# meilisearch/meilisearch

Measured on NVIDIA H100. Metric: queries/sec (batch=1024, typo-tolerant keyword + 768-d cosine hybrid search, semanticRatio 0.5, top-20), higher is better.
Workload: dtype u64+f16/f32

## Files before the change

include/b200milli.h:

```cpp
#ifndef B200MILLI_H
#define B200MILLI_H
#include <stdint.h>
#ifdef __cplusplus
extern "C" {
#endif

#define B200_OK 0
#define B200_ERR_NO_DEVICE (-1)
#define B200_ERR_CUDA (-2)
#define B200_ERR_INVALID (-3)
#define B200_ERR_UNSUPPORTED (-4)
#define B200_ERR_CAPACITY (-5)
#define B200_ERR_STATE (-6)

typedef struct b200_index b200_index;

int b200_open(int device_ordinal, b200_index **out);
void b200_close(b200_index *);
const char *b200_last_error(const b200_index *);
const char *b200_open_error(void);

enum b200_db {
    B200_DB_WORD_DOCIDS = 0,
    B200_DB_EXACT_WORD_DOCIDS = 1,
// ... 161 lines not shown
void b200_rule_end(b200_rule *);

enum b200_kernel { B200_K_LEV = 0, B200_K_COMPACT = 1, B200_K_PAIR_PROBE = 2, B200_K_SCATTER = 3, B200_K_EVAL_PATHS = 4, B200_K_EMIT = 5,
                   B200_K_VEC_DIST = 6, B200_K_TOPK = 7, B200_K_VEC_GEMM = 8, B200_K_VEC_MERGE = 9, B200_K_SORT = 10, B200_K_GEO = 11,
                   B200_K_GEO_FILTER = 12, B200_K_FACET = 13, B200_K_FACET_SEARCH = 14, B200_K_COUNT = 15 };
typedef struct {
    uint64_t kernel_launches;
    uint64_t device_steps;
    uint64_t posting_bytes;
    uint64_t matrix_bytes;
    uint64_t dictionary_bytes;
    uint64_t vector_bytes;
    double kernel_ms[B200_K_COUNT];
    uint64_t kernel_count[B200_K_COUNT];
    uint64_t kernel_bytes[B200_K_COUNT];
    double device_ms;
    uint64_t h2d_bytes, d2h_bytes;
    double host_ms[8];
    uint64_t hbm_bytes_staged;
    uint64_t deferred;
    uint64_t arena_peak_bytes;
    uint64_t eval_class_launches[9];
    uint64_t eval_class_tiles[9];
} b200_stats;
int b200_get_stats(b200_index *, b200_stats *out);
int b200_reset_stats(b200_index *);

#ifdef __cplusplus
}
#endif
#endif
```

meilisearch_b200/__init__.py:

```python
from __future__ import annotations

import ctypes as C
import os
import subprocess

import numpy as np

from .tokenizer import TokenBatch, tokenize

_HERE = os.path.dirname(os.path.abspath(__file__))
LIB_PATH = os.path.join(_HERE, "libb200milli.so")
MAX_SCORES = 12
CRITERIA = {"words": 0, "typo": 1, "proximity": 2, "attribute": 3, "attributeRank": 4, "wordPosition": 5, "sort": 6, "exactness": 7}
DEFAULT_CRITERIA = ["words", "typo", "proximity", "attributeRank", "sort", "wordPosition", "exactness"]
TMS = {"last": 0, "all": 1, "frequency": 2}
SCORE_KINDS = ["words", "typo", "proximity", "fid", "position", "exactAttribute", "exactWords", "vector", "skipped", "sort", "geo"]
GEO_STRATEGIES = {"dynamic": 0, "iterative": 1, "rtree": 2}
DB_FACET_F64, DB_FACET_STRING = 10, 11
DB_FACET_NORMALIZED, DB_FACET_ORIGINALS = 12, 13
NO_FIELD = 0xFFFF
ERRORS = {-1: "NO_DEVICE", -2: "CUDA", -3: "INVALID", -4: "UNSUPPORTED", -5: "CAPACITY", -6: "STATE"}


class B200Error(RuntimeError):
# ... 17 lines not shown
                ("ranking_score_threshold", C.c_double), ("sort_begin", C.c_void_p), ("sort_fid", C.c_void_p), ("sort_asc", C.c_void_p),
                ("sort_geo", C.c_void_p), ("sort_geo_point", C.c_void_p), ("geo_strategy", C.c_int32), ("geo_cache_size", C.c_uint32),
                ("geo_max_bucket_size", C.c_uint64), ("geo_filter_begin", C.c_void_p), ("geo_filter_kind", C.c_void_p),
                ("geo_filter_not", C.c_void_p), ("geo_filter_args", C.c_void_p), ("facet_begin", C.c_void_p), ("facet_fid", C.c_void_p),
                ("facet_order", C.c_void_p), ("facet_max_values", C.c_uint32), ("facet_cap", C.c_uint32), ("facet_search_fid", C.c_void_p),
                ("facet_query_kind", C.c_void_p), ("facet_query_off", C.c_void_p), ("facet_query_bytes", C.c_void_p),
                ("facet_search_flags", C.c_void_p), ("facet_search_max", C.c_uint32)]


class _Results(C.Structure):
    _fields_ = [(n, C.c_void_p) for n in ("docids", "n_hits", "n_scores", "score_kind", "score_rank", "score_max", "score_sim",
                                          "n_candidates", "semantic_hits", "status", "degraded", "used_negative_operator", "candidates")] + \
               [("candidates_words", C.c_uint64)] + \
               [(n, C.c_void_p) for n in ("facet_n_num", "facet_n_str", "facet_key", "facet_count", "facet_docid", "facet_has_stats", "facet_min",
                                          "facet_max")] + \
               [(n, C.c_void_p) for n in ("fs_n", "fs_key", "fs_count", "fs_docid", "fs_fallback")]


class _Stats(C.Structure):
    _fields_ = [("kernel_launches", C.c_uint64), ("device_steps", C.c_uint64), ("posting_bytes", C.c_uint64), ("matrix_bytes", C.c_uint64),
                ("dictionary_bytes", C.c_uint64), ("vector_bytes", C.c_uint64), ("kernel_ms", C.c_double * 15),
                ("kernel_count", C.c_uint64 * 15), ("kernel_bytes", C.c_uint64 * 15), ("device_ms", C.c_double), ("h2d_bytes", C.c_uint64), ("d2h_bytes", C.c_uint64), ("host_ms", C.c_double * 8),
                ("hbm_bytes_staged", C.c_uint64), ("deferred", C.c_uint64), ("arena_peak_bytes", C.c_uint64),
                ("eval_class_launches", C.c_uint64 * 9), ("eval_class_tiles", C.c_uint64 * 9)]


KERNELS = ["lev_match", "act_compact", "pair_probe", "scatter", "eval_paths", "emit", "vec_dist", "topk_select", "vec_gemm_topk", "vec_merge", "sort", "geo", "geo_filter", "facet", "facet_search"]


def build_library(force=False):
    csrc = os.path.join(_HERE, "csrc")
    srcs = [os.path.join(csrc, f) for f in os.listdir(csrc) if f.endswith((".cu", ".cpp", ".h"))] + [os.path.join(_HERE, "..", "include", "b200milli.h")]
    if force or not os.path.exists(LIB_PATH) or any(os.path.getmtime(s) > os.path.getmtime(LIB_PATH) for s in srcs):
        subprocess.check_call(["sh", os.path.join(csrc, "build.sh")])
    return LIB_PATH


_lib = None


def load_library():
    global _lib
    if _lib is None:
        if not os.path.exists(LIB_PATH):
            raise ImportError(f"{LIB_PATH} is missing: run `python -c 'import __graft_entry__ as g; g.build()'` (no CPU fallback exists)")
        l = C.CDLL(LIB_PATH)
        l.b200_open.argtypes = [C.c_int, C.POINTER(C.c_void_p)]
# ... 735 lines not shown
```

meilisearch_b200/csrc/device_types.h:

```cpp
#pragma once
#include <cstdint>

namespace b200 {

struct DListRef {
    unsigned long long off;
    uint32_t card;
    uint32_t dense;
};

constexpr int LEV_MAX_Q = 64;
constexpr int LEV_TERMS_PER_CTA = 32;
constexpr int LEV_REC_CAP = 2048;
struct LevTerm {
    uint8_t q[LEV_MAX_Q];
    uint8_t len;
    int8_t k_same;
    int8_t k_diff;
    uint8_t prefix;
};
struct LevRec {
    uint32_t base;
    uint32_t pad;
    unsigned long long codes;
};

constexpr uint32_t MAX_COSTS = 128;
constexpr uint32_t JOB_CHUNK = 2048;

struct DpState {
    uint32_t edge_begin;
    uint32_t pair_off;
    uint16_t n_edges;
    uint16_t rmin, rcount;
    uint16_t pad;
};
struct DpEdge {
    uint16_t dst;
    uint16_t cost;
    uint16_t col;
    uint16_t pad;
};
constexpr uint32_t MAX_WALK = 14;
struct PathOut {
    uint32_t act;
    uint16_t cost_idx;
    uint16_t len;
// ... 184 lines not shown
```

meilisearch_b200/csrc/engine.h:

```cpp
#pragma once
#include <cuda_runtime.h>

#include <chrono>
#include <condition_variable>
#include <functional>
#include <map>
#include <mutex>
#include <thread>
#include <atomic>
#include <memory>
#include <string>
#include <vector>

#include <sched.h>

#include "../../include/b200milli.h"
#include "device_types.h"
#include "host_index.h"
#include "query_model.h"

namespace b200 {

struct DeviceIndex {
    uint8_t *dict_bytes = nullptr;
// ... 375 lines not shown
    uint8_t *arena = nullptr;
    size_t arena_bytes = 0;
    uint8_t *scratch = nullptr;
    size_t scratch_bytes = 0;
    DevBuf<uint32_t> d_docids_out;
    DevBuf<SortDesc> d_sort_desc;
    DevBuf<uint32_t> d_sort_keys, d_sort_info;
    GeoPoint *d_geo_pts = nullptr;
    unsigned long long *d_geo_ub = nullptr;
    DevBuf<GeoCount> d_geo_count;
    DevBuf<GeoDesc> d_geo_desc;
    DevBuf<uint32_t> d_geo_u32;
    DevBuf<double> d_geo_dist;
    DevBuf<unsigned long long> d_geo_key;
    DevBuf<GeoClause> d_gf_clause;
    DevBuf<GeoFirst> d_gf_first;
    DevBuf<uint32_t> d_gf_u32;
    DevBuf<GeoSlot> d_gf_slot;
    DevBuf<unsigned long long> d_gf_count, d_gf_caller, d_gf_univ;
    DevBuf<unsigned long long> d_universes;
    DevBuf<uint32_t> d_rowtab;
    DevBuf<LevTerm> d_lev_terms;
    DevBuf<LevRec> d_lev_recs;
    DevBuf<uint32_t> d_lev_u32;
    DevBuf<float> d_vq, d_vdist, d_vsel_dist;
    DevBuf<uint32_t> d_vsel_ids, d_vsel_n;
    DevBuf<unsigned long long> d_cand, d_vruns, d_vpartial;
    DevBuf<uint16_t> d_vq16;
    std::vector<cudaEvent_t> ev_pool;
    struct Timed { int cls; size_t a, b; };
    std::vector<Timed> timed;
    size_t ev_used = 0;
    size_t mark();
    void time_kernel(int cls, size_t a, size_t b, uint64_t bytes) {
        timed.push_back(Timed{cls, a, b});
        stats.kernel_count[cls]++;
        stats.kernel_bytes[cls] += bytes;
        stats.kernel_launches++;
    }
    void resolve_timers();

    std::mutex err_mu;
    int fail(int code, const std::string &msg) {
        std::lock_guard<std::mutex> g(err_mu);
        last_error = msg;
        return code;
// ... 82 lines not shown
```

meilisearch_b200/csrc/engine_stage.cpp:

```cpp
#include <cuda_fp16.h>
#include <dlfcn.h>

#include <algorithm>
#include <cctype>
#include <cmath>
#include <cstdio>
#include <cstdlib>
#include <cstring>
#include <stdexcept>

#include "engine.h"
#include "kernels.h"

namespace b200 {

void HostAffinity::detect(int device) {
    valid = false;
    if (const char *env = getenv("B200_PIN"))
        if (atoi(env) == 0) return;
    char bus[32] = {};
    if (cudaDeviceGetPCIBusId(bus, sizeof bus, device) != cudaSuccess) return;
    for (char *c = bus; *c; c++) *c = (char)tolower((unsigned char)*c);
    int node = -1;
    {
// ... 75 lines not shown
    d_facet_out.release();
    d_facet_cand.release();
    if (d_geo_pts) cudaFree(d_geo_pts);
    if (d_geo_ub) cudaFree(d_geo_ub);
    d_geo_count.release();
    d_geo_desc.release();
    d_geo_u32.release();
    d_geo_dist.release();
    d_geo_key.release();
    d_gf_clause.release();
    d_gf_first.release();
    d_gf_u32.release();
    d_gf_slot.release();
    d_gf_count.release();
    d_gf_caller.release();
    d_gf_univ.release();
    for (auto &ln : lanes) ln.release();
    d_docids_out.release();
    d_sort_desc.release();
    d_sort_keys.release();
    d_sort_info.release();
    d_lev_terms.release();
    d_lev_recs.release();
    d_lev_u32.release();
    d_vq.release();
    d_vdist.release();
    d_vsel_dist.release();
    d_vsel_ids.release();
    d_vsel_n.release();
    d_cand.release();
    for (auto e : ev_pool) cudaEventDestroy(e);
    if (sc.comm && sc.comm_destroy) sc.comm_destroy(sc.comm);
    d_gather_ids.release();
    d_gather_dist.release();
    d_gather_n.release();
    for (auto e : vt.ev_pool) cudaEventDestroy(e);
    if (vt.stream) cudaStreamDestroy(vt.stream);
    if (stream) cudaStreamDestroy(stream);
}

size_t Engine::mark() {
    if (ev_used == ev_pool.size()) {
        cudaEvent_t e;
        cudaEventCreate(&e);
        ev_pool.push_back(e);
    }
    cudaEventRecord(ev_pool[ev_used], stream);
    return ev_used++;
}
void Engine::resolve_timers() {
    for (auto &t : timed) {
        float ms = 0;
        if (cudaEventElapsedTime(&ms, ev_pool[t.a], ev_pool[t.b]) == cudaSuccess) stats.kernel_ms[t.cls] += ms;
    }
    timed.clear();
    ev_used = 0;
}

int Engine::stage_finish() {
    CU(cudaSetDevice(device), "cudaSetDevice");
    try {
        build_host_index(raw_dict_bytes, raw_dict_off, raw_dbs, raw_docids, hix);
        build_sort_fields(raw_dbs[B200_DB_FACET_ID_F64_DOCIDS], raw_dbs[B200_DB_FACET_ID_STRING_DOCIDS], hix);
        build_geo_field(raw_dbs[B200_DB_FACET_ID_F64_DOCIDS], raw_dbs[B200_DB_FACET_ID_STRING_DOCIDS], hix);
        build_facet_search(raw_dbs[B200_DB_FACET_ID_STRING_DOCIDS], raw_dbs[B200_DB_FACET_ID_NORMALIZED_STRING_STRINGS],
                           raw_dbs[B200_DB_FIELD_ID_DOCID_FACET_STRINGS], hix);
    } catch (const std::exception &e) {
        return fail(B200_ERR_INVALID, e.what());
    }
    Settings keep = hix.settings;
    (void)keep;
    std::vector<uint32_t> off32(hix.dict_off.size());
    for (size_t i = 0; i < off32.size(); i++) off32[i] = (uint32_t)hix.dict_off[i];
    if (off32.empty()) off32.push_back(0);
    CU(upload(&dix.dict_bytes, hix.dict_bytes.data(), hix.dict_bytes.size()), "upload dictionary");
    CU(upload(&dix.dict_off, off32.data(), off32.size()), "upload dictionary offsets");
    CU(upload(&dix.pool, hix.pool.data(), hix.pool.size()), "upload posting pool");
    static_assert(sizeof(ListRef) == sizeof(DListRef), "ListRef layout");
    CU(upload(&dix.lists, reinterpret_cast<const DListRef *>(hix.lists.data()), hix.lists.size()), "upload list table");
    CU(upload(&dix.pair_keys, reinterpret_cast<const unsigned long long *>(hix.pair_keys.data()), hix.pair_keys.size()), "upload pair keys");
    CU(upload(&dix.base_ub, reinterpret_cast<const unsigned long long *>(hix.base_ub.data()), hix.base_ub.size()), "upload universe");
    stats.hbm_bytes_staged = hix.dict_bytes.size() + off32.size() * 4 + hix.pool.size() * 4 + hix.lists.size() * sizeof(ListRef) +
                             hix.pair_keys.size() * 8 + hix.base_ub.size() * 8;
    std::vector<uint32_t>().swap(hix.pool);
    for (auto &kv : hix.sort_fields)
// ... 114 lines not shown
        CU(cudaMemcpyAsync(dix.emb_docids, docids, n * 4, cudaMemcpyHostToDevice, stream), "H2D embedding docids");
    else {
        std::vector<uint32_t> ids(n);
        for (uint64_t r = 0; r < n; r++) ids[r] = (uint32_t)r;
        CU(cudaMemcpy(dix.emb_docids, ids.data(), n * 4, cudaMemcpyHostToDevice), "H2D embedding docids");
    }
    CU(cudaStreamSynchronize(stream), "sync");
    emb_bitmap.assign(hix.n_words64, 0);
    for (uint64_t r = 0; r < n; r++) {
        const uint32_t doc = docids ? docids[r] : (uint32_t)r;
        if ((doc >> 6) < emb_bitmap.size()) emb_bitmap[doc >> 6] |= 1ull << (doc & 63);
    }
    dix.emb_n = n;
    dix.emb_d = d;
    stats.hbm_bytes_staged += n * d * 2 + n * 8;
    return B200_OK;
}

int Engine::derive_batch(uint32_t n, const char *words, const uint32_t *off, const uint8_t *max_typo, const uint8_t *is_prefix,
                         uint32_t *one_out, uint32_t *n_one, uint32_t *two_out, uint32_t *n_two) {
    if (!staged) return fail(B200_ERR_STATE, "derive before b200_stage_finish");
    CU(cudaSetDevice(device), "cudaSetDevice");
    if (n == 0) return B200_OK;
    std::vector<LevTerm> terms(n);
    for (uint32_t i = 0; i < n; i++) {
        uint32_t len = off[i + 1] - off[i];
        if (len == 0 || len > LEV_MAX_Q) return fail(B200_ERR_UNSUPPORTED, "derive: word longer than 64 bytes (or empty)");
        LevTerm &t = terms[i];
        memset(&t, 0, sizeof t);
        memcpy(t.q, words + off[i], len);
        t.len = (uint8_t)len;
        t.k_same = max_typo[i] >= 2 ? 2 : 1;
        t.k_diff = max_typo[i] >= 2 ? 1 : -1;
        t.prefix = is_prefix[i] ? 1 : 0;
        if (max_typo[i] == 0) t.k_same = -1;
    }
    CU(d_lev_terms.reserve(n), "alloc lev terms");
    CU(d_lev_recs.reserve((size_t)n * LEV_REC_CAP), "alloc lev records");
    size_t per = 1 + 150 + 1 + 50 + 1 + 1;
    CU(d_lev_u32.reserve((size_t)n * per), "alloc lev outputs");
    uint32_t *rec_count = d_lev_u32.p, *d_one = rec_count + n, *d_n_one = d_one + (size_t)n * 150, *d_two = d_n_one + n,
             *d_n_two = d_two + (size_t)n * 50;
    int32_t *d_status = reinterpret_cast<int32_t *>(d_n_two + n);
    CU(cudaMemcpyAsync(d_lev_terms.p, terms.data(), n * sizeof(LevTerm), cudaMemcpyHostToDevice, stream), "H2D lev terms");
    stats.h2d_bytes += n * sizeof(LevTerm);
    stats.d2h_bytes += (size_t)n * (150 + 50 + 3) * 4;
    size_t m0 = mark();
    CU(launch_lev(stream, dix.dict_bytes, dix.dict_off, (uint32_t)hix.n_words, d_lev_terms.p, n, d_lev_recs.p, rec_count, d_one, d_n_one, d_two,
                  d_n_two, d_status),
       "lev kernels");
    size_t m1 = mark();
    uint64_t lev_bytes = (uint64_t)((n + LEV_TERMS_PER_CTA - 1) / LEV_TERMS_PER_CTA) * (hix.dict_bytes.size() + 4 * hix.n_words);
    time_kernel(B200_K_LEV, m0, m1, lev_bytes);
    stats.kernel_launches += 1;
    stats.dictionary_bytes += lev_bytes;
    std::vector<int32_t> status(n);
    CU(cudaMemcpyAsync(one_out, d_one, (size_t)n * 150 * 4, cudaMemcpyDeviceToHost, stream), "D2H");
    CU(cudaMemcpyAsync(n_one, d_n_one, (size_t)n * 4, cudaMemcpyDeviceToHost, stream), "D2H");
    CU(cudaMemcpyAsync(two_out, d_two, (size_t)n * 50 * 4, cudaMemcpyDeviceToHost, stream), "D2H");
    CU(cudaMemcpyAsync(n_two, d_n_two, (size_t)n * 4, cudaMemcpyDeviceToHost, stream), "D2H");
    CU(cudaMemcpyAsync(status.data(), d_status, (size_t)n * 4, cudaMemcpyDeviceToHost, stream), "D2H");
    CU(cudaStreamSynchronize(stream), "sync");
    resolve_timers();
    for (uint32_t i = 0; i < n; i++)
        if (status[i] != 0) return fail(B200_ERR_CAPACITY, "derive: match-record capacity exceeded for a term");
    return B200_OK;
}

int Engine::comm_load() {
    if (sc.lib) return B200_OK;
    void *lib = dlopen("libnccl.so.2", RTLD_NOW | RTLD_NOLOAD);
    if (!lib) lib = dlopen("libnccl.so.2", RTLD_NOW);
    if (!lib) return fail(B200_ERR_STATE, std::string("cannot load libnccl.so.2: ") + dlerror());
    sc.get_unique_id = reinterpret_cast<int (*)(void *)>(dlsym(lib, "ncclGetUniqueId"));
    sc.comm_init_rank = reinterpret_cast<int (*)(void **, int, NcclId, int)>(dlsym(lib, "ncclCommInitRank"));
// ... 329 lines not shown
```

meilisearch_b200/csrc/host_index.h:

```cpp
#pragma once
#include <cstdint>
#include <cstring>
#include <map>
#include <string>
#include <unordered_map>
#include <vector>

namespace b200 {

struct ListRef {
    uint64_t off;
    uint32_t card;
    uint32_t dense;
};

struct RawDb {
    uint64_t n = 0;
    std::vector<uint8_t> keys, vals;
    std::vector<uint64_t> koff, voff;
};

struct Settings {
    uint32_t n_fields = 1;
    std::vector<uint16_t> weights{0};
// ... 35 lines not shown
    std::vector<double> lat, lng;
    std::vector<uint64_t> ub;
    uint64_t n_geo = 0;
};

struct FacetSearchField {
    uint32_t h0 = 0, h1 = 0;
    uint32_t k0 = 0, n_str = 0;
    uint32_t n_entries = 0;
    uint32_t list0 = 0;
};
struct FacetSearchIndex {
    std::map<uint16_t, FacetSearchField> fields;
    std::vector<uint32_t> chars, char_off{0}, csr_off{0}, csr_key;
    std::vector<uint32_t> min_doc;
    std::vector<uint8_t> has_orig;
    std::vector<std::string> orig, key;
};

struct HostIndex {
    std::vector<uint8_t> dict_bytes;
    std::vector<uint64_t> dict_off;
    uint64_t n_words = 0;
    uint32_t n_docs = 0;
    uint32_t n_words64 = 0;
    std::vector<uint64_t> base_ub;
    uint64_t n_documents = 0;
    std::vector<ListRef> lists;
    std::vector<uint32_t> pool;
    std::vector<uint32_t> wd_list, ewd_list;
    std::vector<uint32_t> wf_off, wf_list, wp_off, wp_list;
    std::vector<uint16_t> wf_fid, wp_pos;
    std::vector<std::string> prefixes;
    std::vector<uint32_t> pd_list, epd_list;
    std::vector<uint32_t> pf_off, pf_list, pp_off, pp_list;
    std::vector<uint16_t> pf_fid, pp_pos;
    std::vector<uint64_t> pair_keys;
    uint32_t pair_list_base = 0;
    std::map<uint32_t, uint32_t> fwc_list;
    std::map<uint16_t, SortField> sort_fields;
    GeoField geo;
    FacetSearchIndex fsearch;
    uint32_t db_first[10] = {0}, db_keys[10] = {0};

    Settings settings;

// ... 95 lines not shown
```

meilisearch_b200/csrc/kernels.cu:

```cuda
#include <cuda_fp16.h>
#include <cuda_runtime.h>

#include <cstdint>

#include "device_types.h"
#include "kernels.h"
#include "osa.cuh"

#include <algorithm>

namespace b200 {

constexpr int LEV_TERM_GROUP = 8;
__global__ void __launch_bounds__(256) lev_match_kernel(const uint8_t *__restrict__ dict_bytes, const uint32_t *__restrict__ dict_off,
                                                        uint32_t n_words, const LevTerm *__restrict__ terms, uint32_t n_terms,
                                                        LevRec *__restrict__ recs, uint32_t *__restrict__ rec_count) {
    __shared__ LevTerm sterms[LEV_TERMS_PER_CTA];
    __shared__ uint32_t sterm_sig[LEV_TERMS_PER_CTA], sterm_meta[LEV_TERMS_PER_CTA];
    __shared__ uint8_t sbytes[8192];
    __shared__ uint16_t s_woff[257];
    __shared__ uint32_t s_queue[LEV_TERM_GROUP * 256];
    __shared__ uint32_t s_qn;
    __shared__ unsigned long long s_codes[LEV_TERM_GROUP][8];
    uint32_t w0 = blockIdx.x * 256;
    uint32_t wn = min(256u, n_words - w0);
    uint32_t byte0 = dict_off[w0], byte1 = dict_off[w0 + wn];
    bool in_smem = (byte1 - byte0) <= sizeof(sbytes);
    if (in_smem) {
        for (uint32_t i = threadIdx.x; i < byte1 - byte0; i += blockDim.x) sbytes[i] = dict_bytes[byte0 + i];
        for (uint32_t i = threadIdx.x; i <= wn; i += blockDim.x) s_woff[i] = (uint16_t)(dict_off[w0 + i] - byte0);
    }
    __syncthreads();
    uint32_t wid = w0 + threadIdx.x;
    bool valid = threadIdx.x < wn;
    uint32_t off = valid ? dict_off[wid] : byte0;
    int n = valid ? (int)(dict_off[wid + 1] - off) : 0;
    const uint8_t *w = in_smem ? (sbytes + (off - byte0)) : (dict_bytes + off);
    uint8_t w0c = n > 0 ? w[0] : 0, w1c = n > 1 ? w[1] : 0;
    const uint32_t wsig = char_signature(w, n);
    const uint32_t n_chunks = (n_terms + LEV_TERMS_PER_CTA - 1) / LEV_TERMS_PER_CTA;
    for (uint32_t chunk = blockIdx.y; chunk < n_chunks; chunk += gridDim.y) {
    const uint32_t t0 = chunk * LEV_TERMS_PER_CTA;
    const uint32_t nt = min((uint32_t)LEV_TERMS_PER_CTA, n_terms - t0);
    __syncthreads();
    {
        const uint32_t *src = reinterpret_cast<const uint32_t *>(terms + t0);
        uint32_t *dst = reinterpret_cast<uint32_t *>(sterms);
        for (uint32_t i = threadIdx.x; i < nt * sizeof(LevTerm) / 4; i += blockDim.x) dst[i] = src[i];
    }
    __syncthreads();
    if (threadIdx.x < nt) {
        const LevTerm &T = sterms[threadIdx.x];
        sterm_sig[threadIdx.x] = char_signature(T.q, T.len);
        sterm_meta[threadIdx.x] = (uint32_t)T.len | ((uint32_t)(T.k_same + 1) << 8) | ((uint32_t)(T.k_diff + 1) << 12) |
                                  ((uint32_t)(T.prefix ? 1 : 0) << 16) | ((uint32_t)T.q[0] << 24);
    }
    for (uint32_t tg = 0; tg < nt; tg += LEV_TERM_GROUP) {
        const uint32_t ng = min((uint32_t)LEV_TERM_GROUP, nt - tg);
        if (threadIdx.x == 0) s_qn = 0;
        if (threadIdx.x < LEV_TERM_GROUP * 8) s_codes[threadIdx.x >> 3][threadIdx.x & 7] = 0;
        __syncthreads();
        if (valid && n > 0) {
            for (uint32_t t = 0; t < ng; t++) {
                const uint32_t tsig = sterm_sig[tg + t];
                const uint32_t meta = sterm_meta[tg + t];
                const int kmax = (int)((meta >> 8) & 15) - 1;
                if (__popc(tsig & ~wsig) > kmax) continue;
                const bool prefix = (meta >> 16) & 1;
                const bool sf = (uint8_t)(meta >> 24) == w0c;
                const int k = sf ? kmax : (int)((meta >> 12) & 15) - 1;
                if (k < 0) continue;
                const int m = (int)(meta & 255);
                bool ok = prefix ? (n >= m - k) : (n >= m - k && n <= m + k);
                ok = ok && __popc(tsig & ~wsig) <= k && (prefix || __popc(wsig & ~tsig) <= k);
                if (ok && !sf && m >= 2) {
                    const LevTerm &T = sterms[tg + t];
                    ok = (w1c == T.q[1]) || (w1c == T.q[0]) || (w0c == T.q[1]);
                }
                if (ok) s_queue[atomicAdd(&s_qn, 1u)] = (t << 16) | threadIdx.x | (sf ? 0x80000000u : 0u);
            }
        }
        __syncthreads();
        const uint32_t qn = s_qn;
        for (uint32_t i = threadIdx.x; i < qn; i += blockDim.x) {
            const uint32_t e = s_queue[i];
            const uint32_t t = (e >> 16) & 0x7fff, wi = e & 0xffff;
            const bool sf = (e >> 31) != 0;
            const LevTerm &T = sterms[tg + t];
            const int k = sf ? T.k_same : T.k_diff;
            const uint8_t *ww;
            int wl;
            if (in_smem) {
                ww = sbytes + s_woff[wi];
                wl = (int)s_woff[wi + 1] - (int)s_woff[wi];
            } else {
                uint32_t o = dict_off[w0 + wi];
                ww = dict_bytes + o;
                wl = (int)(dict_off[w0 + wi + 1] - o);
            }
            int d = banded_osa(T.q, T.len, ww, wl, k, T.prefix != 0);
            if (d <= k && d > 0) {
                unsigned long long code = sf ? (unsigned long long)d : 3ull;
                atomicOr(&s_codes[t][wi >> 5], code << (2 * (wi & 31)));
            }
        }
        __syncthreads();
        if (threadIdx.x < ng * 8) {
            const uint32_t t = threadIdx.x >> 3, g = threadIdx.x & 7;
            const unsigned long long codes = s_codes[t][g];
            if (codes) {
                uint32_t slot = atomicAdd(&rec_count[t0 + tg + t], 1u);
                if (slot < LEV_REC_CAP) {
                    LevRec r;
                    r.base = w0 + g * 32;
                    r.pad = 0;
                    r.codes = codes;
                    recs[(size_t)(t0 + tg + t) * LEV_REC_CAP + slot] = r;
                }
            }
        }
        __syncthreads();
    }
    }
}

__global__ void lev_finalize_kernel(LevRec *__restrict__ recs, const uint32_t *__restrict__ rec_count, const LevTerm *__restrict__ terms,
                                    uint32_t n_terms, uint32_t *__restrict__ one_out, uint32_t *__restrict__ n_one,
                                    uint32_t *__restrict__ two_out, uint32_t *__restrict__ n_two, int32_t *__restrict__ status) {
    uint32_t t = blockIdx.x * blockDim.x + threadIdx.x;
    if (t >= n_terms) return;
    uint32_t cnt = rec_count[t];
    if (cnt > LEV_REC_CAP) {
        status[t] = -5;
        cnt = LEV_REC_CAP;
    } else
        status[t] = 0;
    LevRec *r = recs + (size_t)t * LEV_REC_CAP;
    for (uint32_t i = 1; i < cnt; i++) {
        LevRec x = r[i];
        uint32_t j = i;
        while (j > 0 && r[j - 1].base > x.base) {
            r[j] = r[j - 1];
            j--;
        }
        r[j] = x;
    }
    bool two_budget = terms[t].k_same >= 2;
    uint32_t c1 = 0, c2 = 0;
    uint32_t *o1 = one_out + (size_t)t * 150, *o2 = two_out + (size_t)t * 50;
    for (uint32_t i = 0; i < cnt; i++) {
        unsigned long long codes = r[i].codes;
        for (int l = 0; l < 32 && codes; l++, codes >>= 2) {
            int code = (int)(codes & 3);
            if (!code) continue;
            uint32_t wid = r[i].base + l;
            if (!two_budget) {
                if (code == 1 && c1 < 150) o1[c1++] = wid;
                continue;
            }
            bool fin1 = c1 >= 150, fin2 = c2 >= 50;
            if (fin1 && fin2) break;
            if (code == 3 && !fin2) {
                o2[c2++] = wid;
                continue;
            }
            int d = (code == 2) ? 2 : 1;
            if (d == 1) {
                if (!fin1) o1[c1++] = wid;
// ... 1105 lines not shown
cudaError_t launch_shard_merge(cudaStream_t s, const uint32_t *g_ids, const float *g_dist, const uint32_t *g_n, uint32_t world, uint32_t n_q,
                               uint32_t k, uint32_t *out_ids, float *out_dist, uint32_t *out_n) {
    if (!n_q) return cudaSuccess;
    uint32_t cap = 1;
    while (cap < world * k) cap <<= 1;
    const size_t smem = (size_t)cap * 8;
    if (smem > 200 * 1024) return cudaErrorInvalidValue;
    static bool attr_done = false;
    if (!attr_done) {
        cudaError_t e = cudaFuncSetAttribute(shard_merge_kernel, cudaFuncAttributeMaxDynamicSharedMemorySize, 200 * 1024);
        if (e != cudaSuccess) return e;
        attr_done = true;
    }
    shard_merge_kernel<<<n_q, 256, smem, s>>>(g_ids, g_dist, g_n, world, n_q, k, cap, out_ids, out_dist, out_n);
    return cudaGetLastError();
}

#define CK(x)                          \
    do {                               \
        cudaError_t e_ = (x);          \
        if (e_ != cudaSuccess) return e_; \
    } while (0)

cudaError_t launch_lev(cudaStream_t s, const uint8_t *dict_bytes, const uint32_t *dict_off, uint32_t n_words, const LevTerm *terms,
                       uint32_t n_terms, LevRec *recs, uint32_t *rec_count, uint32_t *one_out, uint32_t *n_one, uint32_t *two_out,
                       uint32_t *n_two, int32_t *status) {
    if (n_terms == 0 || n_words == 0) return cudaSuccess;
    CK(cudaMemsetAsync(rec_count, 0, sizeof(uint32_t) * n_terms, s));
    const uint32_t n_chunks = (n_terms + LEV_TERMS_PER_CTA - 1) / LEV_TERMS_PER_CTA;
    dim3 grid((n_words + 255) / 256, n_chunks < 8 ? n_chunks : 8);
    lev_match_kernel<<<grid, 256, 0, s>>>(dict_bytes, dict_off, n_words, terms, n_terms, recs, rec_count);
    lev_finalize_kernel<<<(n_terms + 63) / 64, 64, 0, s>>>(recs, rec_count, terms, n_terms, one_out, n_one, two_out, n_two, status);
    return cudaGetLastError();
}

cudaError_t launch_compact(cudaStream_t s, const CompactTile *tiles, uint32_t n_tiles, bool multi_segment, const ActDesc *acts,
                           uint32_t *seg_count, uint32_t *results) {
    if (!n_tiles) return cudaSuccess;
    if (multi_segment) act_count_kernel<<<n_tiles, COMPACT_THREADS, 0, s>>>(tiles, acts, seg_count);
    act_compact_kernel<<<n_tiles, COMPACT_THREADS, 0, s>>>(tiles, acts, seg_count, results);
    return cudaGetLastError();
}
cudaError_t launch_pair_probe(cudaStream_t s, const PairSet *sets, uint32_t n_sets, uint32_t n_probes, const uint32_t *wordpool,
                              const unsigned long long *pair_keys, uint64_t n_pairs, uint32_t pair_list_base, const DListRef *lists,
                              const ActDesc *acts, const uint32_t *results, Job *queue, uint32_t *qcount, uint32_t qcap) {
    if (!n_probes) return cudaSuccess;
    pair_probe_kernel<<<(n_probes + 255) / 256, 256, 0, s>>>(sets, n_sets, n_probes, wordpool, pair_keys, n_pairs, pair_list_base, lists, acts,
                                                             results, queue, qcount, qcap);
    return cudaGetLastError();
}
cudaError_t launch_scatter(cudaStream_t s, uint32_t n_ctas, const Job *queue, uint32_t *qcount, uint32_t qcap, const ActDesc *acts,
                           const uint32_t *results, const DListRef *lists, const uint32_t *pool, uint32_t *bigq) {
    scatter_kernel<<<n_ctas, 256, 0, s>>>(queue, qcount, qcap, acts, results, lists, pool, bigq);
    scatter_big_kernel<<<n_ctas, 256, 0, s>>>(queue, qcount, acts, results, lists, pool, bigq);
// ... 77 lines not shown
```

meilisearch_b200/csrc/kernels.h:

```cpp
#pragma once
#include <cuda_runtime.h>

#include "device_types.h"

namespace b200 {
cudaError_t launch_lev(cudaStream_t s, const uint8_t *dict_bytes, const uint32_t *dict_off, uint32_t n_words, const LevTerm *terms,
                       uint32_t n_terms, LevRec *recs, uint32_t *rec_count, uint32_t *one_out, uint32_t *n_one, uint32_t *two_out,
                       uint32_t *n_two, int32_t *status);
cudaError_t launch_compact(cudaStream_t s, const CompactTile *tiles, uint32_t n_tiles, bool multi_segment, const ActDesc *acts,
                           uint32_t *seg_count, uint32_t *results);
cudaError_t launch_pair_probe(cudaStream_t s, const PairSet *sets, uint32_t n_sets, uint32_t n_probes, const uint32_t *wordpool,
                              const unsigned long long *pair_keys, uint64_t n_pairs, uint32_t pair_list_base, const DListRef *lists,
                              const ActDesc *acts, const uint32_t *results, Job *queue, uint32_t *qcount, uint32_t qcap);
cudaError_t launch_scatter(cudaStream_t s, uint32_t n_ctas, const Job *queue, uint32_t *qcount, uint32_t qcap, const ActDesc *acts,
                           const uint32_t *results, const DListRef *lists, const uint32_t *pool, uint32_t *bigq);
cudaError_t launch_eval(cudaStream_t s, int cls, const TileDesc *tiles, uint32_t n_tiles, const ActDesc *acts, uint32_t *results,
                        const ColOp *colprog, const uint16_t *costpool, const uint32_t *progpool, unsigned long long *tile_summary);
cudaError_t launch_walk(cudaStream_t s, int cls, const TileDesc *tiles, uint32_t n_tiles, const ActDesc *acts, uint32_t *results,
                        const ColOp *colprog, const DpState *states, const DpEdge *edges, const uint16_t *costpool, const uint32_t *progpool,
                        const unsigned long long *tile_summary, PathOut *pathbuf, uint32_t *path_count, uint32_t path_cap);
cudaError_t launch_emit(cudaStream_t s, const EmitDesc *emits, uint32_t n_emits);
cudaError_t launch_sort_window(cudaStream_t s, const SortDesc *descs, uint32_t n_descs);
cudaError_t launch_geo_count(cudaStream_t s, const GeoCount *counts, uint32_t n);
cudaError_t launch_geo_window(cudaStream_t s, const GeoDesc *descs, uint32_t n_descs);
cudaError_t launch_geo_first_fail(cudaStream_t s, const unsigned long long *geo, const GeoPoint *pts, uint32_t n_words, const GeoClause *clauses,
                                  const uint32_t *radius, uint32_t n_radius, GeoFirst *first);
cudaError_t launch_geo_filter(cudaStream_t s, const unsigned long long *geo, const GeoPoint *pts, uint32_t n_words, const GeoClause *clauses,
                              const GeoFirst *first, const uint32_t *slot_clauses, const GeoSlot *slots, uint32_t n_slots);
cudaError_t launch_facet(cudaStream_t s, const FacetSlot *slots, uint32_t n_slots, uint32_t n_words, uint32_t n_docs);
cudaError_t launch_facet_search_match(cudaStream_t s, const FsTables &t, const FsReq *reqs, uint32_t n, const uint32_t *q_chars);
// ... 31 lines not shown
```

Measured before the change: 12430.

## Prune Levenshtein dictionary scan using first/second-character prefix ranges

Replaces the brute-force scan of every dictionary word against every typo term with work items covering only dictionary ranges whose first or second byte can match the term under the typo budget. Host-side prefix tables (first byte and byte pair lower bounds) are built at staging time. Each term is assigned to disjoint ownership families so each word is counted once, and the finalize pass now merges duplicate record bases. This cuts dictionary bytes scanned and edit-distance evaluations, at the cost of host-side item construction per batch, extra H2D transfers and more record slots.

```diff
diff --git a/include/b200milli.h b/include/b200milli.h
--- a/include/b200milli.h
+++ b/include/b200milli.h
@@ -207,6 +207,9 @@
     uint64_t arena_peak_bytes;
     uint64_t eval_class_launches[9];
     uint64_t eval_class_tiles[9];
+    uint64_t lev_terms;
+    uint64_t lev_items;
+    uint64_t lev_pairs;
 } b200_stats;
 int b200_get_stats(b200_index *, b200_stats *out);
 int b200_reset_stats(b200_index *);
diff --git a/meilisearch_b200/__init__.py b/meilisearch_b200/__init__.py
--- a/meilisearch_b200/__init__.py
+++ b/meilisearch_b200/__init__.py
@@ -63,7 +63,8 @@
                 ("dictionary_bytes", C.c_uint64), ("vector_bytes", C.c_uint64), ("kernel_ms", C.c_double * 15),
                 ("kernel_count", C.c_uint64 * 15), ("kernel_bytes", C.c_uint64 * 15), ("device_ms", C.c_double), ("h2d_bytes", C.c_uint64), ("d2h_bytes", C.c_uint64), ("host_ms", C.c_double * 8),
                 ("hbm_bytes_staged", C.c_uint64), ("deferred", C.c_uint64), ("arena_peak_bytes", C.c_uint64),
-                ("eval_class_launches", C.c_uint64 * 9), ("eval_class_tiles", C.c_uint64 * 9)]
+                ("eval_class_launches", C.c_uint64 * 9), ("eval_class_tiles", C.c_uint64 * 9),
+                ("lev_terms", C.c_uint64), ("lev_items", C.c_uint64), ("lev_pairs", C.c_uint64)]
 
 
 KERNELS = ["lev_match", "act_compact", "pair_probe", "scatter", "eval_paths", "emit", "vec_dist", "topk_select", "vec_gemm_topk", "vec_merge", "sort", "geo", "geo_filter", "facet", "facet_search"]
diff --git a/meilisearch_b200/csrc/device_types.h b/meilisearch_b200/csrc/device_types.h
--- a/meilisearch_b200/csrc/device_types.h
+++ b/meilisearch_b200/csrc/device_types.h
@@ -12,6 +12,8 @@
 constexpr int LEV_MAX_Q = 64;
 constexpr int LEV_TERMS_PER_CTA = 32;
 constexpr int LEV_REC_CAP = 2048;
+constexpr int LEV_MAX_RANGES = 2 + 2 * 254;
+constexpr int LEV_REC_SLOTS = LEV_REC_CAP + LEV_MAX_RANGES;
 struct LevTerm {
     uint8_t q[LEV_MAX_Q];
     uint8_t len;
@@ -23,6 +25,20 @@
     uint32_t base;
     uint32_t pad;
     unsigned long long codes;
+};
+enum LevFamily : uint32_t {
+    LEV_F1 = 0,
+    LEV_F2A = 1,
+    LEV_F2B = 2,
+    LEV_F3 = 3,
+    LEV_F0 = 4,
+};
+constexpr int LEV_FAMILY_SHIFT = 29;
+struct LevItem {
+    uint32_t lo;
+    uint32_t t_off;
+    uint16_t n;
+    uint16_t t_cnt;
 };
 
 constexpr uint32_t MAX_COSTS = 128;
diff --git a/meilisearch_b200/csrc/engine.h b/meilisearch_b200/csrc/engine.h
--- a/meilisearch_b200/csrc/engine.h
+++ b/meilisearch_b200/csrc/engine.h
@@ -421,6 +421,10 @@
     DevBuf<uint32_t> d_rowtab;
     DevBuf<LevTerm> d_lev_terms;
     DevBuf<LevRec> d_lev_recs;
+    DevBuf<LevItem> d_lev_items;
+    DevBuf<uint32_t> d_lev_perm;
+    std::vector<LevItem> lev_items;
+    std::vector<uint32_t> lev_perm;
     DevBuf<uint32_t> d_lev_u32;
     DevBuf<float> d_vq, d_vdist, d_vsel_dist;
     DevBuf<uint32_t> d_vsel_ids, d_vsel_n;
diff --git a/meilisearch_b200/csrc/engine_stage.cpp b/meilisearch_b200/csrc/engine_stage.cpp
--- a/meilisearch_b200/csrc/engine_stage.cpp
+++ b/meilisearch_b200/csrc/engine_stage.cpp
@@ -121,6 +121,8 @@
     d_sort_info.release();
     d_lev_terms.release();
     d_lev_recs.release();
+    d_lev_items.release();
+    d_lev_perm.release();
     d_lev_u32.release();
     d_vq.release();
     d_vdist.release();
@@ -156,10 +158,30 @@
     ev_used = 0;
 }
 
+static void build_prefix_tables(HostIndex &ix) {
+    if (ix.n_words >= (1ull << 32)) throw std::runtime_error("dictionary: more than 2^32 - 1 words");
+    for (uint64_t i = 1; i < ix.n_words; i++)
+        if (ix.cmp_word(i - 1, ix.word_ptr(i), ix.word_len(i)) >= 0)
+            throw std::runtime_error("dictionary: words are not in strictly ascending bytewise order at word " + std::to_string(i));
+    ix.first_lo.resize(257);
+    ix.pair_lo.resize(65537);
+    for (uint32_t c = 0; c < 256; c++) {
+        const uint8_t k[1] = {(uint8_t)c};
+        ix.first_lo[c] = (uint32_t)ix.lower_bound(k, 1);
+    }
+    ix.first_lo[256] = (uint32_t)ix.n_words;
+    for (uint32_t p = 0; p < 65536; p++) {
+        const uint8_t k[2] = {(uint8_t)(p >> 8), (uint8_t)p};
+        ix.pair_lo[p] = (uint32_t)ix.lower_bound(k, 2);
+    }
+    ix.pair_lo[65536] = (uint32_t)ix.n_words;
+}
+
 int Engine::stage_finish() {
     CU(cudaSetDevice(device), "cudaSetDevice");
     try {
         build_host_index(raw_dict_bytes, raw_dict_off, raw_dbs, raw_docids, hix);
+        build_prefix_tables(hix);
         build_sort_fields(raw_dbs[B200_DB_FACET_ID_F64_DOCIDS], raw_dbs[B200_DB_FACET_ID_STRING_DOCIDS], hix);
         build_geo_field(raw_dbs[B200_DB_FACET_ID_F64_DOCIDS], raw_dbs[B200_DB_FACET_ID_STRING_DOCIDS], hix);
         build_facet_search(raw_dbs[B200_DB_FACET_ID_STRING_DOCIDS], raw_dbs[B200_DB_FACET_ID_NORMALIZED_STRING_STRINGS],
@@ -320,6 +342,7 @@
     if (!staged) return fail(B200_ERR_STATE, "derive before b200_stage_finish");
     CU(cudaSetDevice(device), "cudaSetDevice");
     if (n == 0) return B200_OK;
+    if (n >= (1u << LEV_FAMILY_SHIFT)) return fail(B200_ERR_UNSUPPORTED, "derive: too many terms in one batch");
     std::vector<LevTerm> terms(n);
     for (uint32_t i = 0; i < n; i++) {
         uint32_t len = off[i + 1] - off[i];
@@ -333,22 +356,74 @@
         t.prefix = is_prefix[i] ? 1 : 0;
         if (max_typo[i] == 0) t.k_same = -1;
     }
+    std::vector<uint32_t> by_first[256], by_second[256], whole;
+    for (uint32_t i = 0; i < n; i++) {
+        const LevTerm &t = terms[i];
+        if (t.k_same < 0) continue;
+        by_first[t.q[0]].push_back(i | LEV_F1 << LEV_FAMILY_SHIFT);
+        if (t.k_diff < 0) continue;
+        if (t.len < 2 || t.q[0] == 0 || t.q[1] == 0) {
+            whole.push_back(i | LEV_F0 << LEV_FAMILY_SHIFT);
+            continue;
+        }
+        by_second[t.q[1]].push_back(i | LEV_F2B << LEV_FAMILY_SHIFT);
+        if (t.q[1] != t.q[0]) {
+            by_first[t.q[1]].push_back(i | LEV_F2A << LEV_FAMILY_SHIFT);
+            by_second[t.q[0]].push_back(i | LEV_F3 << LEV_FAMILY_SHIFT);
+        }
+    }
+    lev_perm.clear();
+    lev_items.clear();
+    uint64_t lev_bytes = 0, lev_pairs = 0;
+    auto emit = [&](uint32_t p0, uint32_t cnt, uint32_t lo, uint32_t hi) {
+        for (uint32_t a = lo; a < hi;) {
+            const uint32_t b = std::min(hi, (a & ~255u) + 256);
+            for (uint32_t c = 0; c < cnt; c += LEV_TERMS_PER_CTA) {
+                const uint32_t tc = std::min(cnt - c, (uint32_t)LEV_TERMS_PER_CTA);
+                lev_items.push_back(LevItem{a, p0 + c, (uint16_t)(b - a), (uint16_t)tc});
+                lev_pairs += (uint64_t)(b - a) * tc;
+            }
+            lev_bytes += (uint64_t)((cnt + LEV_TERMS_PER_CTA - 1) / LEV_TERMS_PER_CTA) * (hix.dict_off[b] - hix.dict_off[a] + 4ull * (b - a));
+            a = b;
+        }
+    };
+    auto slots = [&](const std::vector<uint32_t> &v) {
+        lev_perm.insert(lev_perm.end(), v.begin(), v.end());
+        return (uint32_t)(lev_perm.size() - v.size());
+    };
+    for (uint32_t g = 0; g < 256; g++) {
+        if (!by_first[g].empty()) emit(slots(by_first[g]), (uint32_t)by_first[g].size(), hix.first_lo[g], hix.first_lo[g + 1]);
+        if (by_second[g].empty()) continue;
+        const uint32_t p0 = slots(by_second[g]), cnt = (uint32_t)by_second[g].size();
+        for (uint32_t c = 0; c < 256; c++)
+            if (c != g) emit(p0, cnt, hix.pair_lo[c << 8 | g], hix.pair_hi(c, g));
+    }
+    if (!whole.empty()) emit(slots(whole), (uint32_t)whole.size(), 0, (uint32_t)hix.n_words);
+    const uint32_t n_items = (uint32_t)lev_items.size();
     CU(d_lev_terms.reserve(n), "alloc lev terms");
-    CU(d_lev_recs.reserve((size_t)n * LEV_REC_CAP), "alloc lev records");
+    CU(d_lev_items.reserve(n_items), "alloc lev work items");
+    CU(d_lev_perm.reserve(lev_perm.size()), "alloc lev term slots");
+    CU(d_lev_recs.reserve((size_t)n * LEV_REC_SLOTS), "alloc lev records");
     size_t per = 1 + 150 + 1 + 50 + 1 + 1;
     CU(d_lev_u32.reserve((size_t)n * per), "alloc lev outputs");
     uint32_t *rec_count = d_lev_u32.p, *d_one = rec_count + n, *d_n_one = d_one + (size_t)n * 150, *d_two = d_n_one + n,
              *d_n_two = d_two + (size_t)n * 50;
     int32_t *d_status = reinterpret_cast<int32_t *>(d_n_two + n);
     CU(cudaMemcpyAsync(d_lev_terms.p, terms.data(), n * sizeof(LevTerm), cudaMemcpyHostToDevice, stream), "H2D lev terms");
-    stats.h2d_bytes += n * sizeof(LevTerm);
+    if (n_items) {
+        CU(cudaMemcpyAsync(d_lev_items.p, lev_items.data(), n_items * sizeof(LevItem), cudaMemcpyHostToDevice, stream), "H2D lev items");
+        CU(cudaMemcpyAsync(d_lev_perm.p, lev_perm.data(), lev_perm.size() * 4, cudaMemcpyHostToDevice, stream), "H2D lev term slots");
+    }
+    stats.h2d_bytes += n * sizeof(LevTerm) + n_items * sizeof(LevItem) + lev_perm.size() * 4;
     stats.d2h_bytes += (size_t)n * (150 + 50 + 3) * 4;
+    stats.lev_terms += n;
+    stats.lev_items += n_items;
+    stats.lev_pairs += lev_pairs;
     size_t m0 = mark();
-    CU(launch_lev(stream, dix.dict_bytes, dix.dict_off, (uint32_t)hix.n_words, d_lev_terms.p, n, d_lev_recs.p, rec_count, d_one, d_n_one, d_two,
-                  d_n_two, d_status),
+    CU(launch_lev(stream, dix.dict_bytes, dix.dict_off, d_lev_items.p, n_items, d_lev_perm.p, d_lev_terms.p, n, d_lev_recs.p, rec_count, d_one,
+                  d_n_one, d_two, d_n_two, d_status),
        "lev kernels");
     size_t m1 = mark();
-    uint64_t lev_bytes = (uint64_t)((n + LEV_TERMS_PER_CTA - 1) / LEV_TERMS_PER_CTA) * (hix.dict_bytes.size() + 4 * hix.n_words);
     time_kernel(B200_K_LEV, m0, m1, lev_bytes);
     stats.kernel_launches += 1;
     stats.dictionary_bytes += lev_bytes;
diff --git a/meilisearch_b200/csrc/host_index.h b/meilisearch_b200/csrc/host_index.h
--- a/meilisearch_b200/csrc/host_index.h
+++ b/meilisearch_b200/csrc/host_index.h
@@ -81,6 +81,9 @@
     std::vector<uint8_t> dict_bytes;
     std::vector<uint64_t> dict_off;
     uint64_t n_words = 0;
+    std::vector<uint32_t> first_lo;
+    std::vector<uint32_t> pair_lo;
+    uint32_t pair_hi(uint32_t c, uint32_t g) const { return g < 255 ? pair_lo[(c << 8 | g) + 1] : first_lo[c + 1]; }
     uint32_t n_docs = 0;
     uint32_t n_words64 = 0;
     std::vector<uint64_t> base_ub;
diff --git a/meilisearch_b200/csrc/kernels.cu b/meilisearch_b200/csrc/kernels.cu
--- a/meilisearch_b200/csrc/kernels.cu
+++ b/meilisearch_b200/csrc/kernels.cu
@@ -12,48 +12,60 @@
 namespace b200 {
 
 constexpr int LEV_TERM_GROUP = 8;
+__device__ __forceinline__ bool lev_owns(uint32_t own, uint8_t w0c, uint8_t w1c) {
+    const uint8_t q0 = (uint8_t)own, q1 = (uint8_t)(own >> 8);
+    switch (own >> 16) {
+        case LEV_F1: return w0c == q0;
+        case LEV_F2A: return w0c == q1 && q1 != q0;
+        case LEV_F2B: return w1c == q1 && w0c != q0 && w0c != q1;
+        case LEV_F3: return w1c == q0 && q0 != q1 && w0c != q0 && w0c != q1;
+        default: return w0c != q0;
+    }
+}
 __global__ void __launch_bounds__(256) lev_match_kernel(const uint8_t *__restrict__ dict_bytes, const uint32_t *__restrict__ dict_off,
-                                                        uint32_t n_words, const LevTerm *__restrict__ terms, uint32_t n_terms,
-                                                        LevRec *__restrict__ recs, uint32_t *__restrict__ rec_count) {
+                                                        const LevItem *__restrict__ items, const uint32_t *__restrict__ perm,
+                                                        const LevTerm *__restrict__ terms, LevRec *__restrict__ recs,
+                                                        uint32_t *__restrict__ rec_count) {
     __shared__ LevTerm sterms[LEV_TERMS_PER_CTA];
-    __shared__ uint32_t sterm_sig[LEV_TERMS_PER_CTA], sterm_meta[LEV_TERMS_PER_CTA];
+    __shared__ uint32_t sterm_sig[LEV_TERMS_PER_CTA], sterm_meta[LEV_TERMS_PER_CTA], sterm_own[LEV_TERMS_PER_CTA], sterm_id[LEV_TERMS_PER_CTA];
     __shared__ uint8_t sbytes[8192];
     __shared__ uint16_t s_woff[257];
     __shared__ uint32_t s_queue[LEV_TERM_GROUP * 256];
     __shared__ uint32_t s_qn;
     __shared__ unsigned long long s_codes[LEV_TERM_GROUP][8];
-    uint32_t w0 = blockIdx.x * 256;
-    uint32_t wn = min(256u, n_words - w0);
-    uint32_t byte0 = dict_off[w0], byte1 = dict_off[w0 + wn];
-    bool in_smem = (byte1 - byte0) <= sizeof(sbytes);
+    const LevItem item = items[blockIdx.x];
+    const uint32_t tile = item.lo & ~255u, a = item.lo - tile;
+    const uint32_t nt = item.t_cnt;
+    const uint32_t byte0 = dict_off[item.lo], byte1 = dict_off[item.lo + item.n];
+    const bool in_smem = (byte1 - byte0) <= sizeof(sbytes);
     if (in_smem) {
         for (uint32_t i = threadIdx.x; i < byte1 - byte0; i += blockDim.x) sbytes[i] = dict_bytes[byte0 + i];
-        for (uint32_t i = threadIdx.x; i <= wn; i += blockDim.x) s_woff[i] = (uint16_t)(dict_off[w0 + i] - byte0);
-    }
+        for (uint32_t i = threadIdx.x; i <= item.n; i += blockDim.x) s_woff[i] = (uint16_t)(dict_off[item.lo + i] - byte0);
+    }
+    if (threadIdx.x < nt) sterm_id[threadIdx.x] = perm[item.t_off + threadIdx.x];
     __syncthreads();
-    uint32_t wid = w0 + threadIdx.x;
-    bool valid = threadIdx.x < wn;
+    {
+        constexpr uint32_t W = sizeof(LevTerm) / 4;
+        uint32_t *dst = reinterpret_cast<uint32_t *>(sterms);
+        for (uint32_t i = threadIdx.x; i < nt * W; i += blockDim.x) {
+            const uint32_t t = sterm_id[i / W] & ((1u << LEV_FAMILY_SHIFT) - 1);
+            dst[i] = reinterpret_cast<const uint32_t *>(terms + t)[i % W];
+        }
+    }
+    const uint32_t wid = tile + threadIdx.x;
+    const bool valid = threadIdx.x >= a && threadIdx.x < a + item.n;
     uint32_t off = valid ? dict_off[wid] : byte0;
     int n = valid ? (int)(dict_off[wid + 1] - off) : 0;
     const uint8_t *w = in_smem ? (sbytes + (off - byte0)) : (dict_bytes + off);
     uint8_t w0c = n > 0 ? w[0] : 0, w1c = n > 1 ? w[1] : 0;
+    __syncthreads();
     const uint32_t wsig = char_signature(w, n);
-    const uint32_t n_chunks = (n_terms + LEV_TERMS_PER_CTA - 1) / LEV_TERMS_PER_CTA;
-    for (uint32_t chunk = blockIdx.y; chunk < n_chunks; chunk += gridDim.y) {
-    const uint32_t t0 = chunk * LEV_TERMS_PER_CTA;
-    const uint32_t nt = min((uint32_t)LEV_TERMS_PER_CTA, n_terms - t0);
-    __syncthreads();
-    {
-        const uint32_t *src = reinterpret_cast<const uint32_t *>(terms + t0);
-        uint32_t *dst = reinterpret_cast<uint32_t *>(sterms);
-        for (uint32_t i = threadIdx.x; i < nt * sizeof(LevTerm) / 4; i += blockDim.x) dst[i] = src[i];
-    }
-    __syncthreads();
     if (threadIdx.x < nt) {
         const LevTerm &T = sterms[threadIdx.x];
         sterm_sig[threadIdx.x] = char_signature(T.q, T.len);
         sterm_meta[threadIdx.x] = (uint32_t)T.len | ((uint32_t)(T.k_same + 1) << 8) | ((uint32_t)(T.k_diff + 1) << 12) |
                                   ((uint32_t)(T.prefix ? 1 : 0) << 16) | ((uint32_t)T.q[0] << 24);
+        sterm_own[threadIdx.x] = (uint32_t)T.q[0] | ((uint32_t)T.q[1] << 8) | ((sterm_id[threadIdx.x] >> LEV_FAMILY_SHIFT) << 16);
     }
     for (uint32_t tg = 0; tg < nt; tg += LEV_TERM_GROUP) {
         const uint32_t ng = min((uint32_t)LEV_TERM_GROUP, nt - tg);
@@ -66,6 +78,7 @@
                 const uint32_t meta = sterm_meta[tg + t];
                 const int kmax = (int)((meta >> 8) & 15) - 1;
                 if (__popc(tsig & ~wsig) > kmax) continue;
+                if (!lev_owns(sterm_own[tg + t], w0c, w1c)) continue;
                 const bool prefix = (meta >> 16) & 1;
                 const bool sf = (uint8_t)(meta >> 24) == w0c;
                 const int k = sf ? kmax : (int)((meta >> 12) & 15) - 1;
@@ -91,12 +104,12 @@
             const uint8_t *ww;
             int wl;
             if (in_smem) {
-                ww = sbytes + s_woff[wi];
-                wl = (int)s_woff[wi + 1] - (int)s_woff[wi];
+                ww = sbytes + s_woff[wi - a];
+                wl = (int)s_woff[wi - a + 1] - (int)s_woff[wi - a];
             } else {
-                uint32_t o = dict_off[w0 + wi];
+                uint32_t o = dict_off[tile + wi];
                 ww = dict_bytes + o;
-                wl = (int)(dict_off[w0 + wi + 1] - o);
+                wl = (int)(dict_off[tile + wi + 1] - o);
             }
             int d = banded_osa(T.q, T.len, ww, wl, k, T.prefix != 0);
             if (d <= k && d > 0) {
@@ -109,18 +122,18 @@
             const uint32_t t = threadIdx.x >> 3, g = threadIdx.x & 7;
             const unsigned long long codes = s_codes[t][g];
             if (codes) {
-                uint32_t slot = atomicAdd(&rec_count[t0 + tg + t], 1u);
-                if (slot < LEV_REC_CAP) {
+                const uint32_t term = sterm_id[tg + t] & ((1u << LEV_FAMILY_SHIFT) - 1);
+                uint32_t slot = atomicAdd(&rec_count[term], 1u);
+                if (slot < LEV_REC_SLOTS) {
                     LevRec r;
-                    r.base = w0 + g * 32;
+                    r.base = tile + g * 32;
                     r.pad = 0;
                     r.codes = codes;
-                    recs[(size_t)(t0 + tg + t) * LEV_REC_CAP + slot] = r;
+                    recs[(size_t)term * LEV_REC_SLOTS + slot] = r;
                 }
             }
         }
         __syncthreads();
-    }
     }
 }
 
@@ -130,12 +143,9 @@
     uint32_t t = blockIdx.x * blockDim.x + threadIdx.x;
     if (t >= n_terms) return;
     uint32_t cnt = rec_count[t];
-    if (cnt > LEV_REC_CAP) {
-        status[t] = -5;
-        cnt = LEV_REC_CAP;
-    } else
-        status[t] = 0;
-    LevRec *r = recs + (size_t)t * LEV_REC_CAP;
+    status[t] = cnt > LEV_REC_SLOTS ? -5 : 0;
+    cnt = min(cnt, (uint32_t)LEV_REC_SLOTS);
+    LevRec *r = recs + (size_t)t * LEV_REC_SLOTS;
     for (uint32_t i = 1; i < cnt; i++) {
         LevRec x = r[i];
         uint32_t j = i;
@@ -144,6 +154,18 @@
             j--;
         }
         r[j] = x;
+    }
+    uint32_t u = 0;
+    for (uint32_t i = 0; i < cnt; i++) {
+        if (u > 0 && r[u - 1].base == r[i].base)
+            r[u - 1].codes |= r[i].codes;
+        else
+            r[u++] = r[i];
+    }
+    cnt = u;
+    if (cnt > LEV_REC_CAP) {
+        status[t] = -5;
+        cnt = LEV_REC_CAP;
     }
     bool two_budget = terms[t].k_same >= 2;
     uint32_t c1 = 0, c2 = 0;
@@ -1295,14 +1317,12 @@
         if (e_ != cudaSuccess) return e_; \
     } while (0)
 
-cudaError_t launch_lev(cudaStream_t s, const uint8_t *dict_bytes, const uint32_t *dict_off, uint32_t n_words, const LevTerm *terms,
-                       uint32_t n_terms, LevRec *recs, uint32_t *rec_count, uint32_t *one_out, uint32_t *n_one, uint32_t *two_out,
+cudaError_t launch_lev(cudaStream_t s, const uint8_t *dict_bytes, const uint32_t *dict_off, const LevItem *items, uint32_t n_items,
+                       const uint32_t *perm, const LevTerm *terms, uint32_t n_terms, LevRec *recs, uint32_t *rec_count, uint32_t *one_out, uint32_t *n_one, uint32_t *two_out,
                        uint32_t *n_two, int32_t *status) {
-    if (n_terms == 0 || n_words == 0) return cudaSuccess;
+    if (n_terms == 0) return cudaSuccess;
     CK(cudaMemsetAsync(rec_count, 0, sizeof(uint32_t) * n_terms, s));
-    const uint32_t n_chunks = (n_terms + LEV_TERMS_PER_CTA - 1) / LEV_TERMS_PER_CTA;
-    dim3 grid((n_words + 255) / 256, n_chunks < 8 ? n_chunks : 8);
-    lev_match_kernel<<<grid, 256, 0, s>>>(dict_bytes, dict_off, n_words, terms, n_terms, recs, rec_count);
+    if (n_items) lev_match_kernel<<<n_items, 256, 0, s>>>(dict_bytes, dict_off, items, perm, terms, recs, rec_count);
     lev_finalize_kernel<<<(n_terms + 63) / 64, 64, 0, s>>>(recs, rec_count, terms, n_terms, one_out, n_one, two_out, n_two, status);
     return cudaGetLastError();
 }
diff --git a/meilisearch_b200/csrc/kernels.h b/meilisearch_b200/csrc/kernels.h
--- a/meilisearch_b200/csrc/kernels.h
+++ b/meilisearch_b200/csrc/kernels.h
@@ -4,8 +4,8 @@
 #include "device_types.h"
 
 namespace b200 {
-cudaError_t launch_lev(cudaStream_t s, const uint8_t *dict_bytes, const uint32_t *dict_off, uint32_t n_words, const LevTerm *terms,
-                       uint32_t n_terms, LevRec *recs, uint32_t *rec_count, uint32_t *one_out, uint32_t *n_one, uint32_t *two_out,
+cudaError_t launch_lev(cudaStream_t s, const uint8_t *dict_bytes, const uint32_t *dict_off, const LevItem *items, uint32_t n_items,
+                       const uint32_t *perm, const LevTerm *terms, uint32_t n_terms, LevRec *recs, uint32_t *rec_count, uint32_t *one_out, uint32_t *n_one, uint32_t *two_out,
                        uint32_t *n_two, int32_t *status);
 cudaError_t launch_compact(cudaStream_t s, const CompactTile *tiles, uint32_t n_tiles, bool multi_segment, const ActDesc *acts,
                            uint32_t *seg_count, uint32_t *results);
```

Result: faster. 13310 (median of 6 runs) (+7.0%).
